# adjo0043/Mathematical-Modeling-Of-Infectious-Diseases-V1

Measured on AMD Instinct MI355X. Metric: ODE-solve+likelihood evals/sec (SEPAIHRD 4-age, 400d), higher is better.
Workload: dtype f64

## Files before the change

### mathematical-modeling-of-infectious-diseases-v1_amd/csrc/phase_pass.py

```python
#!/usr/bin/env python3
import argparse, os, re, subprocess, sys, tempfile

LLVM = "/opt/rocm/lib/llvm/bin"
MCPU = "gfx950"
E64_OK = re.compile(r"^\s+(v_fmac_f64_e32|v_mov_b32_e32|v_mov_b64_e32|v_add_u32_e32|v_sub_u32_e32|v_subrev_u32_e32|v_mul_f32_e32|v_add_f32_e32|"
                    r"v_cvt_f32_f64_e32|v_cvt_f64_f32_e32|v_cvt_f64_i32_e32|v_rcp_f64_e32|v_log_f32_e32|v_exp_f32_e32|v_and_b32_e32|v_or_b32_e32|"
                    r"v_lshlrev_b32_e32|v_max_i32_e32|v_min_i32_e32)\b")


def assemble_sizes(path):
    tmp = tempfile.mkdtemp(prefix="pp_")
    obj = os.path.join(tmp, "a.o")
    subprocess.run([LLVM + "/clang", "-x", "assembler", "-target", "amdgcn-amd-amdhsa", "-mcpu=" + MCPU, "-c", path, "-o", obj], check=True,
                   stdout=subprocess.DEVNULL, stderr=subprocess.DEVNULL)
    dis = subprocess.run([LLVM + "/llvm-objdump", "-d", obj], check=True, capture_output=True, text=True).stdout
    out, cur = {}, None
    for line in dis.splitlines():
        m = re.match(r"^[0-9a-f]+ <(\S+)>:", line)
        if m:
            cur = out.setdefault(m.group(1), [])
            continue
        m = re.match(r"^\s+(\S+).*//\s*([0-9A-Fa-f]+):\s+((?:[0-9A-Fa-f]{8}\s*)+)", line)
        if m and cur is not None:
            cur.append((int(m.group(2), 16), 4 * len(m.group(3).split()), m.group(1)))
    return out


def protected_spans(lines, idxs):
    out = set()
    for k, li in enumerate(idxs):
        if not lines[li].strip().startswith("s_getpc_b64"):
            continue
        last = k
        for m in range(k + 1, min(k + 8, len(idxs))):
            if "@rel32" in lines[idxs[m]]:
                last = m
        out.update(range(k + 1, last + 1))
    return out


def off_phase_runs(sizes, wanted, min_run, min_block):
    n_runs = n_off = 0
    for name, ins in sizes.items():
        if not any(w in name for w in wanted):
            continue
        start = 0
        for k in range(len(ins) + 1):
            if not (k == len(ins) or ins[k][2].startswith(("s_cbranch", "s_branch", "s_endpgm", "s_setpc"))):
                continue
            blk = ins[start:min(k + 1, len(ins))]
            start = k + 1
            if len(blk) < min_block:
                continue
            j = 0
            while j < len(blk):
                if blk[j][1] != 8:
                    j += 1
                    continue
                r = j
                while r < len(blk) and blk[r][1] == 8:
                    r += 1
                if r - j >= min_run:
                    n_runs += 1
                    n_off += blk[j][0] % 8 == 4
                j = r
    return n_runs, n_off


def is_instruction(line):
    t = line.strip()
    return bool(t) and not t.startswith((";", ".", "//", "#")) and not re.match(r"^[\w.$]+:", t)


def main():
    global LLVM, MCPU
    ap = argparse.ArgumentParser()
    ap.add_argument("src"); ap.add_argument("dst")
    ap.add_argument("--kernels", default="sepaihrd_eval_quad_kernel,sepaihrd_eval_kernelILi16E")
    ap.add_argument("--min-run", type=int, default=3)
    ap.add_argument("--min-block", type=int, default=200)
    ap.add_argument("--nop-run", type=int, default=7, help="insert s_nop 0 in front of an off-phase run at least this long when nothing can be re-encoded")
    ap.add_argument("--look-back", type=int, default=12)
    ap.add_argument("--body-residue", type=int, default=-1,
                    help="0, 8, .., 56: pad the ENTRY of every sepaihrd_eval_quad_kernel (s_nop pairs, executed once per wave) so that its "
                         "largest straight-line block -- the common RK body -- starts at this offset within a 64-byte line.  The 8-byte phase "
                         "is untouched (pads come in pairs).  Measured (round 4, tools/ab.sh): five instructions fewer in the consumer's "
                         "logarithm moved the body from offset 60 to 20 and cost the headline kernel 1 % at an unchanged phase report")
    ap.add_argument("--llvm", default=LLVM, help="directory of clang / llvm-objdump")
    ap.add_argument("--mcpu", default=MCPU)
    args = ap.parse_args()
    LLVM, MCPU = args.llvm, args.mcpu
    wanted = args.kernels.split(",")
    sizes = assemble_sizes(args.src)
    lines = open(args.src).read().split("\n")
    func, funcs = None, {}
    for i, l in enumerate(lines):
        m = re.match(r"^(\w+):\s*(;.*)?$", l)
        if m and m.group(1) in sizes:
            func = m.group(1); funcs[func] = []
            continue
        if l.startswith("\t.end_amdhsa_kernel") or l.strip().startswith(".Lfunc_end"):
            func = None
        if func is not None and is_instruction(l):
            funcs[func].append(i)
    n_re = n_nop = n_runs = n_fixed = 0
    edits = {}
    inserts = {}
    for name, idxs in funcs.items():
        if not any(w in name for w in wanted):
            continue
        ins = sizes[name]
        if len(ins) != len(idxs):
            print(f"skip {name[:70]}: {len(ins)} disassembled vs {len(idxs)} listed instructions", file=sys.stderr)
            continue
        guarded = protected_spans(lines, idxs)
        start = 0
        shift = 0
        for k in range(len(ins) + 1):
            end_block = k == len(ins) or ins[k][2].startswith(("s_cbranch", "s_branch", "s_endpgm", "s_setpc"))
            if not end_block:
                continue
            blk = list(range(start, min(k + 1, len(ins))))
            start = k + 1
            if len(blk) < args.min_block:
                continue
            j = 0
            last_touch = -1
            while j < len(blk):
                a = blk[j]
                if ins[a][1] != 8:
                    j += 1
                    continue
                r = j
                while r < len(blk) and ins[blk[r]][1] == 8:
                    r += 1
                run_len = r - j
                if run_len >= args.min_run:
                    n_runs += 1
                    if (ins[a][0] + shift) % 8 == 4:
                        fixed = False
                        for b in range(j - 1, max(j - 1 - args.look_back, last_touch), -1):
                            li = idxs[blk[b]]
                            if blk[b] in guarded:
                                continue
                            if ins[blk[b]][1] == 4 and li not in edits and E64_OK.match(lines[li]) and "0x" not in lines[li] and "dpp" not in lines[li] and "sdwa" not in lines[li]:
                                edits[li] = lines[li].replace("_e32", "_e64", 1)
                                shift += 4; n_re += 1; fixed = True; last_touch = b
                                break
                        if not fixed and run_len >= args.nop_run and a not in guarded:
                            inserts[idxs[a]] = "\ts_nop 0"
                            shift += 4; n_nop += 1; fixed = True; last_touch = j
                        n_fixed += fixed
                j = r
    out = []
    for i, l in enumerate(lines):
        if i in inserts:
            out.append(inserts[i])
        out.append(edits.get(i, l))
    open(args.dst, "w").write("\n".join(out))
    try:
        after = assemble_sizes(args.dst)
    except subprocess.CalledProcessError:
        print("phase_pass: the rewritten assembly does not assemble", file=sys.stderr)
        sys.exit(1)
    if args.body_residue >= 0:
        out_lines = open(args.dst).read().split("\n")
        inserts_at = {}
        for name, ins in after.items():
            if "sepaihrd_eval_quad_kernel" not in name or not ins:
                continue
            blocks, start = [], 0
            for k in range(len(ins) + 1):
                if k == len(ins) or ins[k][2].startswith(("s_cbranch", "s_branch", "s_endpgm", "s_setpc")):
                    blocks.append(ins[start:min(k + 1, len(ins))]); start = k + 1
            bodies = [b for b in blocks if len(b) >= args.min_block and sum(1 for _, _, m in b if "f64" in m or "dpp" in m) * 2 > len(b)]
            if not bodies:
                continue
            body = min(bodies, key=len)
            delta = (args.body_residue - body[0][0]) % 64
            delta -= delta % 8
            if delta:
                inserts_at[name] = delta // 4
        if inserts_at:
            padded = []
            for l in out_lines:
                padded.append(l)
                m = re.match(r"^(\w+):\s*(;.*)?$", l)
                if m and m.group(1) in inserts_at:
                    padded.extend(["\ts_nop 0"] * inserts_at[m.group(1)])
            open(args.dst, "w").write("\n".join(padded))
            try:
                after = assemble_sizes(args.dst)
            except subprocess.CalledProcessError:
                print("phase_pass: the padded assembly does not assemble", file=sys.stderr)
                sys.exit(1)
            print(f"body residue {args.body_residue}: entry pads {sorted(set(inserts_at.values()))} s_nop in {len(inserts_at)} kernels")
    runs_before, off_before = off_phase_runs(sizes, wanted, args.min_run, args.min_block)
    runs_after, off_after = off_phase_runs(after, wanted, args.min_run, args.min_block)
    print(f"runs of >= {args.min_run} wide encodings: {n_runs}; off phase and fixed: {n_fixed} ({n_re} re-encoded, {n_nop} s_nop); "
          f"off-phase runs by the assembled addresses: {off_before} of {runs_before} before, {off_after} of {runs_after} after")
    if off_after > off_before:
        print("phase_pass: the rewritten assembly has MORE off-phase runs than its input", file=sys.stderr)
        sys.exit(1)


if __name__ == "__main__":
    main()
```

### mathematical-modeling-of-infectious-diseases-v1_amd/csrc/sepaihrd_kernels.hip

```cpp
#include <hip/hip_runtime.h>
#include <float.h>
#include <math.h>
#include <stdint.h>
#include <stdlib.h>

#include <mutex>
#include <utility>

#include "sepaihrd_device.h"

#ifndef SEPAIHRD_DOPRI5_WPS2
#define SEPAIHRD_DOPRI5_WPS2 0
#endif
#ifndef SEPAIHRD_LL_STATE_IN_LDS
#define SEPAIHRD_LL_STATE_IN_LDS 1
#endif
#ifndef SEPAIHRD_ARITH_FMA
#error "compile with -DSEPAIHRD_ARITH_FMA=0 or 1"
#endif

namespace sepaihrd {
namespace {

#include "sepaihrd_dev_common.inc"
// ... 91 lines not shown
    dx[3] = fma(-q.get(MF_GAMMA_A), A, q.get(MF_PG) * P);
    dx[4] = fma(-q.get(MF_R_I), I, q.get(MF_PI) * P);
    dx[5] = fma(-q.get(MF_R_H), H, flow_IH);
    dx[6] = fma(-q.get(MF_R_ICU), ICU, flow_H_ICU);
    dx[7] = fma(q.get(MF_GAMMA_ICU), ICU, fma(q.get(MF_GAMMA_A), A, fma(q.get(MF_GAMMA_H), H, q.get(MF_GAMMA_I) * I)));
    dx[8] = fma(q.get(MF_D_ICU), ICU, fma(q.get(MF_D_COMM), I, q.get(MF_D_H) * H));
    dx[9] = flow_IH;
    dx[10] = flow_H_ICU;
#else
    const double flow_EP = q.get(MF_SIGMA) * E;
    const double flow_P_out = q.get(MF_GAMMA_P) * P;
    const double flow_PA = q.get(MF_P) * flow_P_out;
    const double flow_PI = flow_P_out - flow_PA;
    const double flow_IH = q.get(MF_H) * I;
    const double flow_IR = q.get(MF_GAMMA_I) * I;
    const double flow_ID_community = q.get(MF_D_COMM) * I;
    const double flow_H_ICU = q.get(MF_ICU) * H;

    dx[0] = -flow_SE;
    dx[1] = flow_SE - flow_EP;
    dx[2] = flow_EP - flow_P_out;
    dx[3] = flow_PA - q.get(MF_GAMMA_A) * A;
    const double I_out = flow_IR + flow_IH + flow_ID_community;
    const double H_out = q.get(MF_GAMMA_H) * H + q.get(MF_D_H) * H + flow_H_ICU;
    const double ICU_out = (q.get(MF_GAMMA_ICU) + q.get(MF_D_ICU)) * ICU;
    dx[4] = flow_PI - I_out;
    dx[5] = flow_IH - H_out;
    dx[6] = flow_H_ICU - ICU_out;
    dx[7] = q.get(MF_GAMMA_A) * A + flow_IR + q.get(MF_GAMMA_H) * H + q.get(MF_GAMMA_ICU) * ICU;
    dx[8] = q.get(MF_D_H) * H + q.get(MF_D_ICU) * ICU + flow_ID_community;
    dx[9] = flow_IH;
    dx[10] = flow_H_ICU;
#endif
}

#ifdef SEPAIHRD_STAMPS
#define SEP_STAMP(var)                                                                 \
    do {                                                                               \
        __builtin_amdgcn_sched_barrier(0);                                             \
        asm volatile("s_memtime %0\n\ts_waitcnt lgkmcnt(0)" : "=s"(var)::"memory");     \
        __builtin_amdgcn_sched_barrier(0);                                             \
    } while (0)
#else
#define SEP_STAMP(var) do { } while (0)
#endif

#include "sepaihrd_step_control.inc"

#if SEPAIHRD_ARITH_FMA
enum QuadCoefDopri5 { QD_B32 = 0, QD_B42, QD_B43, QD_B52, QD_B53, QD_B54, QD_B62, QD_B63, QD_B64, QD_B65, QD_C3, QD_C4, QD_C5,
                      QD_C6, QD_DC4, QD_DC5, QD_DC6 , QD_DC7  };
enum QuadCoefCashKarp { QK_A32 = 0, QK_A42, QK_A43, QK_A52, QK_A53, QK_A54, QK_A62, QK_A63, QK_A64, QK_A65, QK_B3, QK_B4, QK_B6,
                        QK_DB4, QK_DB5, QK_DB6 };
__device__ const double QUAD_COEF[2][2][16] = {
    {{dp::b32, dp::b42, dp::b43, dp::b52, dp::b53, dp::b54, dp::b62, dp::b63, dp::b64, dp::b65, dp::c3, dp::c4, dp::c5, dp::c6,
      dp::dc4, dp::dc5},
     {dp::dc6, dp::dc7, 0, 0, 0, 0, 0, 0, 0, 0, 0, 0, 0, 0, 0, 0}},
    {{ck::a32, ck::a42, ck::a43, ck::a52, ck::a53, ck::a54, ck::a62, ck::a63, ck::a64, ck::a65, ck::b3, ck::b4, ck::b6, ck::db4,
      ck::db5, ck::db6},
     {0, 0, 0, 0, 0, 0, 0, 0, 0, 0, 0, 0, 0, 0, 0, 0}}};
template <int IDX>
__device__ __forceinline__ void stage_term(double& acc, double vecA, double vecB, double k) {
    if constexpr (IDX < 16) fmac_row_bcast<IDX, 0xf, false>(acc, vecA, k);
    else fmac_row_bcast<IDX - 16, 0xf, false>(acc, vecB, k);
}


#ifndef SEPAIHRD_FMA16_STAGE_PADS
#define SEPAIHRD_FMA16_STAGE_PADS 194
#endif
#ifndef SEPAIHRD_FMA3_STAGE_PADS
#define SEPAIHRD_FMA3_STAGE_PADS 0
#endif
#define SEP_ROW_STAGE_PAD(i, v) do { if ((((N == NUM_COMP) ? SEPAIHRD_FMA16_STAGE_PADS : (N == 3) ? SEPAIHRD_FMA3_STAGE_PADS : 0) >> (i)) & 1) asm volatile("s_nop 0" : "+v"(v)); } while (0)

template <int SOLVER, int N, class RHS>
__device__ __forceinline__ void rk_stages_row_coef(const double cur, const double vecA, const double vecB, const double (&x)[N],
                                                   double (&k1)[N], double (&k2)[N], double (&k3)[N], double (&k4)[N], double (&k5)[N],
                                                   double (&k6)[N], double (&k7)[N], double (&xnew)[N], double (&xerr)[N],
                                                   const double (&bks)[7], RHS&& rhs_call) {
    double xt[N];
        if (SOLVER == 0) {
            { const double f1 = cur * dp::b21;
              SEP_UNROLL for (int c = 0; c < N; ++c) xt[c] = fma(f1, k1[c], x[c]);
              SEP_ROW_STAGE_PAD(0, xt[0]); rhs_call(xt, k2, bks[1]); }
            SEP_ROW_STAGE_PAD(1, k2[0]);
            { const double f1 = cur * dp::b31;
              SEP_UNROLL for (int c = 0; c < N; ++c) { xt[c] = fma(f1, k1[c], x[c]); stage_term<QD_B32>(xt[c], vecA, vecB, k2[c]); }
              SEP_ROW_STAGE_PAD(2, xt[0]); rhs_call(xt, k3, bks[2]); }
            SEP_ROW_STAGE_PAD(3, k3[0]);
            { const double f1 = cur * dp::b41;
              SEP_UNROLL for (int c = 0; c < N; ++c) {
                  xt[c] = fma(f1, k1[c], x[c]); stage_term<QD_B42>(xt[c], vecA, vecB, k2[c]); stage_term<QD_B43>(xt[c], vecA, vecB, k3[c]); }
              SEP_ROW_STAGE_PAD(4, xt[0]); rhs_call(xt, k4, bks[3]); }
            SEP_ROW_STAGE_PAD(5, k4[0]);
            { const double f1 = cur * dp::b51;
              SEP_UNROLL for (int c = 0; c < N; ++c) {
                  xt[c] = fma(f1, k1[c], x[c]); stage_term<QD_B52>(xt[c], vecA, vecB, k2[c]); stage_term<QD_B53>(xt[c], vecA, vecB, k3[c]);
                  stage_term<QD_B54>(xt[c], vecA, vecB, k4[c]); }
              SEP_ROW_STAGE_PAD(6, xt[0]); rhs_call(xt, k5, bks[4]); }
            SEP_ROW_STAGE_PAD(7, k5[0]);
            { const double f1 = cur * dp::b61;
              SEP_UNROLL for (int c = 0; c < N; ++c) {
                  xt[c] = fma(f1, k1[c], x[c]); stage_term<QD_B62>(xt[c], vecA, vecB, k2[c]); stage_term<QD_B63>(xt[c], vecA, vecB, k3[c]);
                  stage_term<QD_B64>(xt[c], vecA, vecB, k4[c]); stage_term<QD_B65>(xt[c], vecA, vecB, k5[c]); }
              SEP_ROW_STAGE_PAD(8, xt[0]); rhs_call(xt, k6, bks[5]); }
            SEP_ROW_STAGE_PAD(9, k6[0]);
            { const double f1 = cur * dp::c1;
              SEP_UNROLL for (int c = 0; c < N; ++c) {
                  xnew[c] = fma(f1, k1[c], x[c]); stage_term<QD_C3>(xnew[c], vecA, vecB, k3[c]); stage_term<QD_C4>(xnew[c], vecA, vecB, k4[c]);
                  stage_term<QD_C5>(xnew[c], vecA, vecB, k5[c]); stage_term<QD_C6>(xnew[c], vecA, vecB, k6[c]); }
              SEP_ROW_STAGE_PAD(10, xnew[0]); rhs_call(xnew, k7, bks[6]); }
            SEP_ROW_STAGE_PAD(11, k7[0]);
            { const double e1 = cur * dp::dc1, e3 = cur * dp::dc3;
              SEP_UNROLL for (int c = 0; c < N; ++c) {
                  xerr[c] = fma(e1, k1[c], e3 * k3[c]); stage_term<QD_DC4>(xerr[c], vecA, vecB, k4[c]); stage_term<QD_DC5>(xerr[c], vecA, vecB, k5[c]);
                  stage_term<QD_DC6>(xerr[c], vecA, vecB, k6[c]); stage_term<QD_DC7>(xerr[c], vecA, vecB, k7[c]); } }
        } else {
            rhs_call(x, k1, bks[0]);
            { const double f1 = ck::a21 * cur;
              SEP_UNROLL for (int c = 0; c < N; ++c) xt[c] = fma(f1, k1[c], x[c]);
              rhs_call(xt, k2, bks[1]); }
            { const double f1 = ck::a31 * cur;
              SEP_UNROLL for (int c = 0; c < N; ++c) { xt[c] = fma(f1, k1[c], x[c]); stage_term<QK_A32>(xt[c], vecA, vecB, k2[c]); }
              rhs_call(xt, k3, bks[2]); }
            { const double f1 = ck::a41 * cur;
              SEP_UNROLL for (int c = 0; c < N; ++c) {
// ... 1040 lines not shown
```

### mathematical-modeling-of-infectious-diseases-v1_amd/csrc/sepaihrd_lane_split.inc

```

constexpr int QUAD_LANES = 16;
constexpr int QUAD_CPW = WAVE / QUAD_LANES;
constexpr int QUAD_SLOTS = 3;

template <int CTRL>
__device__ __forceinline__ double quad_rot(double v) { return dpp_move<CTRL>(v); }
constexpr int QROT_LEFT = 0x93;
constexpr int QROT_NEXT = 0x39;

#ifndef SEPAIHRD_STRICT_STAGE_PADS
#define SEPAIHRD_STRICT_STAGE_PADS 0
#endif
#define SEP_STAGE_PAD(i, v) do { if ((SEPAIHRD_STRICT_STAGE_PADS >> (i)) & 1) asm volatile("s_nop 0" : "+v"(v)); } while (0)
#ifndef SEPAIHRD_STRICT_HEAD_PADS_CK
#define SEPAIHRD_STRICT_HEAD_PADS_CK 0
#endif
#ifndef SEPAIHRD_STRICT_STAGE_PADS_CK
#define SEPAIHRD_STRICT_STAGE_PADS_CK 0
#endif
#define SEP_STAGE_PAD_CK(i, v) do { if ((SEPAIHRD_STRICT_STAGE_PADS_CK >> (i)) & 1) asm volatile("s_nop 0" : "+v"(v)); } while (0)
#define SEP_PHASE_PAD(n) do { if ((n) >= 1) asm volatile("s_nop 0"); if ((n) >= 2) asm volatile("s_nop 0"); if ((n) >= 3) asm volatile("s_nop 0"); } while (0)
using lanemask = unsigned long long;
__device__ __forceinline__ lanemask lanes_where(bool p) { return __builtin_amdgcn_ballot_w64(p); }
__device__ __forceinline__ bool lane_of(lanemask m) { return __builtin_amdgcn_inverse_ballot_w64(m); }
__device__ __forceinline__ double min_plain(double a, double b) {
    double r;
    asm("v_min_f64 %0, %1, %2" : "=v"(r) : "v"(a), "v"(b));
    return r;
}

#if SEPAIHRD_ARITH_FMA
struct QuadModel {
    double theta_inf, m[4];
    double cO1, cL1;
    double cO0, cX0, cL0;
    double a1, a2, a3, a4, a5;
};

__device__ __forceinline__ void rhs_quad(const QuadModel& q, const double (&x)[QUAD_SLOTS], double (&dx)[QUAD_SLOTS],
                                         double beta_eff) {
    const double Lx1 = quad_rot<QROT_LEFT>(x[1]);
    const double Nx1 = quad_rot<QROT_NEXT>(x[1]), Nx0 = quad_rot<QROT_NEXT>(x[0]);
    const double pressure = fma(q.theta_inf, x[1], Lx1 + x[0]);
    double lambda = 0.0;
    fmac_row_bcast<2, 0xf, true>(lambda, pressure, q.m[0]);
    fmac_row_bcast<6, 0xf, false>(lambda, pressure, q.m[1]);
    fmac_row_bcast<10, 0xf, false>(lambda, pressure, q.m[2]);
    fmac_row_bcast<14, 0xf, false>(lambda, pressure, q.m[3]);
    lambda *= beta_eff;
    const double lambda_val = (0.0 < lambda) ? lambda : 0.0;
    const double W = lambda_val * x[0];
    dx[1] = fma(q.cO1, x[1], fma(q.cL1, Lx1, W));
    dx[0] = fma(q.cO0, x[0], fma(q.cX0, x[1], fma(q.cL0, Lx1, -W)));
    dx[2] = fma(q.a5, Nx0, fma(q.a4, x[0], fma(q.a3, Lx1, fma(q.a2, Nx1, q.a1 * x[1]))));
}

#else
struct QuadModel {
    double theta_inf, h_infec, inv_N, a_i, m[4];
    double u2, u3, v1, v2, v3;
    double u5, u6, u7, w1;
    double q1, q2, q3, q4, q5, q6;
};

__device__ __forceinline__ void rhs_quad(const QuadModel& q, const double (&x)[QUAD_SLOTS], double (&dx)[QUAD_SLOTS],
                                         double beta_eff) {
    const double Lx1 = quad_rot<QROT_LEFT>(x[1]);
    const double Nx1 = quad_rot<QROT_NEXT>(x[1]), Nx0 = quad_rot<QROT_NEXT>(x[0]);
    const double total_inf = Lx1 + x[0] + q.theta_inf * x[1];
    const double pressure = total_inf * q.h_infec * q.inv_N;
    double lambda = q.m[0] * dpp_bcast_row<2, 0xf, 2, 0x0>(pressure);
    lambda += q.m[1] * dpp_bcast_row<6, 0xf, 6, 0x0>(pressure);
    lambda += q.m[2] * dpp_bcast_row<10, 0xf, 10, 0x0>(pressure);
    lambda += q.m[3] * dpp_bcast_row<14, 0xf, 14, 0x0>(pressure);
    lambda *= beta_eff * q.a_i;
    const double lambda_val = (0.0 < lambda) ? lambda : 0.0;
    const double W = lambda_val * x[0];
    {
        const double t = q.u2 * Lx1;
        const double flow_in = (W + t) - q.u3 * t;
        const double out = q.v1 * x[1] + q.v2 * x[1] + q.v3 * x[1];
        dx[1] = flow_in - out;
    }
    {
        const double t5 = q.u5 * Lx1;
        const double flow_in = q.u6 * t5 + q.u7 * x[1];
        dx[0] = (flow_in - q.w1 * x[0]) - W;
    }
    dx[2] = q.q1 * x[0] + q.q2 * x[1] + q.q3 * Nx1 + q.q4 * Nx0 + q.q5 * x[0] + q.q6 * Lx1;
}

#endif

__device__ __forceinline__ int quad_comp(int cg, int slot) {
    if (slot == 0) return cg == 0 ? 0 : (cg == 1 ? -1 : (cg == 2 ? 3 : 6));
    if (slot == 1) return cg == 0 ? 1 : (cg == 1 ? 2 : (cg == 2 ? 4 : 5));
    return cg == 0 ? 10 : (cg == 1 ? 9 : (cg == 2 ? 7 : 8));
}

constexpr int QUAD_RING = 32;
constexpr int QUAD_BURST = 12;
constexpr int QUAD_UNITS = 4;
constexpr int QUAD_ROW_DOUBLES = QUAD_CPW * 12;
constexpr int QUAD_SPIN_LIMIT = 1 << 22;
constexpr size_t QUAD_FUSED_MAX_LDS = 144 * 1024;
constexpr int QUAD_CTRL_INTS = 8 + QUAD_UNITS * (2 * QUAD_CPW + 1 + 3 * QUAD_CPW);
constexpr int SEPAIHRD_STATUS_PIPELINE = 4;
// ... 364 lines not shown
            } else {
                if (stores) *cum_row = v - prev;
                cum_row += cum_step;
            }
            prev = v;
            if constexpr (TRAJ) {
            if (out.traj != nullptr && chain_valid && age < n_real) {
                double* tdst = out.traj + ((size_t)chain * pb.T + k) * (NUM_COMP * n_real) + age;
                SEP_UNROLL
                for (int s = 0; s < NS; ++s) {
                    const int c = quad_comp(cg, s);
                    if (c >= 0) tdst[c * n_real] = x[s];
                }
            }
            }
        }
    };

    int k_next = 1;
    double t = pb.times[0];
    double dt = pb.dt_hint;
    int fails = 0;
    int attempts = 0;
    double t_next = (T > 1) ? pb.times[1] : t;
    double t_after = (T > 2) ? pb.times[2] : t_next;
    observe_store(act, 0);
    if (T <= 1) act = 0ull;

    sch.lo = INFINITY; sch.hi = -INFINITY; sch.bk = 0.0;
    double k1[NS];
    if (SOLVER == 0) {
        int c0, c1;
        segment_index2(sch, pb.nm_pad, t, t, c0, c1);
        rhs_quad(q, x, k1, sch.bkv[c0]);
    }
    const double eps_abs = pb.abs_tol, eps_rel = pb.rel_tol;
#if SEPAIHRD_ARITH_FMA
    const double coefA = QUAD_COEF[SOLVER][0][lane & 15], coefB = QUAD_COEF[SOLVER][1][lane & 15];
#else
    const double coefA = STRICT_QUAD_COEF[SOLVER][0][lane & 15], coefB = STRICT_QUAD_COEF[SOLVER][1][lane & 15];
#endif

#ifdef SEPAIHRD_STAMPS
    unsigned long long st0 = 0, st1 = 0, st2 = 0, st3 = 0, st4 = 0;
    unsigned long long acc_head = 0, acc_body = 0, acc_err = 0, acc_tail = 0;
#endif
    auto attempt = [&](const double cur, const double vecA, const double vecB, const double (&bks)[7]) __attribute__((always_inline)) {
        const bool active = lane_of(act);
        (void)active;
        SEP_STAMP(st1);
        double k2[NS], k3[NS], k4[NS], k5[NS], k6[NS], k7[NS];
        double xnew[NS], xerr[NS];
#if SEPAIHRD_ARITH_FMA
        rk_stages_row_coef<SOLVER, NS>(cur, vecA, vecB, x, k1, k2, k3, k4, k5, k6, k7, xnew, xerr, bks,
                                       [&](const double (&xin)[NS], double (&kout)[NS], double bk) { rhs_quad(q, xin, kout, bk); });
#else
        double xt[NS];
        if (SOLVER == 0) {
            { const double f1 = strict_coef<SD_B21>(vecA, vecB);
              SEP_UNROLL for (int c = 0; c < NS; ++c) xt[c] = x[c] + f1 * k1[c];
              rhs_quad(q, xt, k2, bks[1]); }
            SEP_STAGE_PAD(0, k2[0]);
            { const double f1 = strict_coef<SD_B31>(vecA, vecB), f2 = strict_coef<SD_B32>(vecA, vecB);
              SEP_UNROLL for (int c = 0; c < NS; ++c) xt[c] = x[c] + f1 * k1[c] + f2 * k2[c];
              rhs_quad(q, xt, k3, bks[2]); }
            SEP_STAGE_PAD(1, k3[0]);
            { const double f1 = strict_coef<SD_B41>(vecA, vecB), f2 = strict_coef<SD_B42>(vecA, vecB), f3 = strict_coef<SD_B43>(vecA, vecB);
              SEP_UNROLL for (int c = 0; c < NS; ++c) xt[c] = x[c] + f1 * k1[c] + f2 * k2[c] + f3 * k3[c];
              rhs_quad(q, xt, k4, bks[3]); }
            SEP_STAGE_PAD(2, k4[0]);
            { const double f1 = strict_coef<SD_B51>(vecA, vecB), f2 = strict_coef<SD_B52>(vecA, vecB), f3 = strict_coef<SD_B53>(vecA, vecB), f4 = strict_coef<SD_B54>(vecA, vecB);
              SEP_UNROLL for (int c = 0; c < NS; ++c)
                  xt[c] = x[c] + f1 * k1[c] + f2 * k2[c] + f3 * k3[c] + f4 * k4[c];
              rhs_quad(q, xt, k5, bks[4]); }
            SEP_STAGE_PAD(3, k5[0]);
            { const double f1 = strict_coef<SD_B61>(vecA, vecB), f2 = strict_coef<SD_B62>(vecA, vecB), f3 = strict_coef<SD_B63>(vecA, vecB), f4 = strict_coef<SD_B64>(vecA, vecB),
                           f5 = strict_coef<SD_B65>(vecA, vecB);
              SEP_UNROLL for (int c = 0; c < NS; ++c)
                  xt[c] = x[c] + f1 * k1[c] + f2 * k2[c] + f3 * k3[c] + f4 * k4[c] + f5 * k5[c];
              rhs_quad(q, xt, k6, bks[5]); }
            SEP_STAGE_PAD(4, k6[0]);
            { const double f1 = strict_coef<SD_C1>(vecA, vecB), f3 = strict_coef<SD_C3>(vecA, vecB), f4 = strict_coef<SD_C4>(vecA, vecB), f5 = strict_coef<SD_C5>(vecA, vecB),
                           f6 = strict_coef<SD_C6>(vecA, vecB);
              SEP_UNROLL for (int c = 0; c < NS; ++c)
                  xnew[c] = x[c] + f1 * k1[c] + f3 * k3[c] + f4 * k4[c] + f5 * k5[c] + f6 * k6[c];
              rhs_quad(q, xnew, k7, bks[6]); }
            SEP_STAGE_PAD(5, k7[0]);
            { const double e1 = strict_coef<SD_DC1>(vecA, vecB), e3 = strict_coef<SD_DC3>(vecA, vecB), e4 = strict_coef<SD_DC4>(vecA, vecB), e5 = strict_coef<SD_DC5>(vecA, vecB),
                           e6 = strict_coef<SD_DC6>(vecA, vecB), e7 = strict_coef<SD_DC7>(vecA, vecB);
              SEP_UNROLL for (int c = 0; c < NS; ++c)
                  xerr[c] = e1 * k1[c] + e3 * k3[c] + e4 * k4[c] + e5 * k5[c] + e6 * k6[c] + e7 * k7[c]; }
        } else {
            rhs_quad(q, x, k1, bks[0]);
            SEP_STAGE_PAD_CK(0, k1[0]);
            { const double f1 = strict_coef<SK_A21>(vecA, vecB);
              SEP_UNROLL for (int c = 0; c < NS; ++c) xt[c] = x[c] + f1 * k1[c];
              rhs_quad(q, xt, k2, bks[1]); }
            SEP_STAGE_PAD_CK(1, k2[0]);
            { const double f1 = strict_coef<SK_A31>(vecA, vecB), f2 = strict_coef<SK_A32>(vecA, vecB);
              SEP_UNROLL for (int c = 0; c < NS; ++c) xt[c] = x[c] + f1 * k1[c] + f2 * k2[c];
              rhs_quad(q, xt, k3, bks[2]); }
            SEP_STAGE_PAD_CK(2, k3[0]);
            { const double f1 = strict_coef<SK_A41>(vecA, vecB), f2 = strict_coef<SK_A42>(vecA, vecB), f3 = strict_coef<SK_A43>(vecA, vecB);
              SEP_UNROLL for (int c = 0; c < NS; ++c) xt[c] = x[c] + f1 * k1[c] + f2 * k2[c] + f3 * k3[c];
              rhs_quad(q, xt, k4, bks[3]); }
            SEP_STAGE_PAD_CK(3, k4[0]);
            { const double f1 = strict_coef<SK_A51>(vecA, vecB), f2 = strict_coef<SK_A52>(vecA, vecB), f3 = strict_coef<SK_A53>(vecA, vecB), f4 = strict_coef<SK_A54>(vecA, vecB);
              SEP_UNROLL for (int c = 0; c < NS; ++c)
// ... 51 lines not shown
            const double cur_after = lane_of(dec_m | inc_m) ? cur * f : cur;
            dt = rej ? cur_after : (acc ? max_moved(dt, cur_after) : dt);
            n_rej += rej ? 1 : 0;
            const lanemask gave_up = dec_m & lanes_where(fails >= 500);
            if (lane_of(gave_up)) status = 2;
            act &= ~gave_up;
            fails = acc ? 0 : fails + (rej ? 1 : 0);
        } else {
            fails = 0;
        }
        n_acc += acc ? 1 : 0;
        SEP_STAMP(st3);
        {
            if (acc) {
                t += cur;
                SEP_UNROLL
                for (int c = 0; c < NS; ++c) x[c] = xnew[c];
                if (SOLVER == 0) {
                    SEP_UNROLL
                    for (int c = 0; c < NS; ++c) k1[c] = k7[c];
                }
            }
            const lanemask reached_m = acc_m & ~lanes_where((t_next - t) > DBL_EPSILON);
            if (__builtin_expect(reached_m != 0ull, 1)) {
                const double t_fetch = lds_times[(k_next + 2 < T) ? k_next + 2 : T - 1];
                observe_store(reached_m, k_next);
                if (lane_of(reached_m)) {
                    t = t_next;
                    ++k_next;
                    t_next = t_after;
                    t_after = t_fetch;
                }
                act &= ~(reached_m & lanes_where(k_next >= T));
            }
        }
        SEP_STAMP(st4);
    };
    while (act != 0ull && attempts < pb.max_attempts) {
#ifdef SEPAIHRD_PHASE_NOPS_HEAD
        SEP_PHASE_PAD(SEPAIHRD_PHASE_NOPS_HEAD);
#endif
#if !SEPAIHRD_ARITH_FMA
        if constexpr (SOLVER == 1) SEP_PHASE_PAD(SEPAIHRD_STRICT_HEAD_PADS_CK);
#endif
        SEP_STAMP(st0);
        double cur_m;
        {
            const double gap = t_next - t;
            asm volatile("v_min_f64 %0, %1, %2" : "=v"(cur_m) : "v"(dt), "v"(gap));
        }
        const double cur = lane_of(act) ? cur_m : 1.0;
#if SEPAIHRD_ARITH_FMA
        double vecA, vecB;
        asm("v_mul_f64 %0, %2, %3\n\tv_mul_f64 %1, %2, %4" : "=&v"(vecA), "=&v"(vecB) : "v"(cur), "v"(coefA), "v"(coefB));
#else
        const double vecA = cur * coefA, vecB = cur * coefB;
#endif
        const double tmin = (SOLVER == 0) ? fma(cur, dp::a2, t) : t;
        const double tmax = (SOLVER == 0) ? t + cur : fma(ck::c5, cur, t);
        const lanemask in_seg = lanes_where(tmin > sch.lo) & lanes_where(tmax <= sch.hi);
        auto stage_values = [&](double (&bks)[7], int c_lo, int c_hi, double v_lo, double v_hi) __attribute__((always_inline)) {
            double tau[7];
            if (SOLVER == 0) {
                tau[0] = t;
                tau[1] = t + cur * dp::a2; tau[2] = t + cur * dp::a3; tau[3] = t + cur * dp::a4;
                tau[4] = t + cur * dp::a5; tau[5] = t + cur; tau[6] = t + cur;
            } else {
                tau[0] = t;
                tau[1] = t + ck::c2 * cur; tau[2] = t + ck::c3 * cur; tau[3] = t + ck::c4 * cur;
                tau[4] = t + ck::c5 * cur; tau[5] = t + ck::c6 * cur; tau[6] = t + cur;
            }
            if (lanes_where(c_hi > c_lo + 1) == 0ull) {
                const double bpt = (c_lo < pb.nm) ? sch.me[c_lo] : INFINITY;
                SEP_UNROLL
                for (int s = 0; s < 7; ++s) bks[s] = (tau[s] > bpt) ? v_hi : v_lo;
            } else {
                for (int s = 0; s < 7; ++s) {
                    int ca, cb;
                    segment_index2(sch, pb.nm_pad, tau[s], tau[s], ca, cb);
                    bks[s] = sch.bkv[ca];
                }
            }
        };
#if SEPAIHRD_ARITH_FMA
        if (__builtin_expect((act & ~in_seg) != 0ull, 0)) {
            int c_lo, c_hi;
            segment_index2(sch, pb.nm_pad, tmin, tmax, c_lo, c_hi);
            const double v_lo = sch.bkv[c_lo], v_hi = sch.bkv[c_hi];
            const lanemask straddles = act & lanes_where(c_hi > c_lo);
            sch.lo = (c_hi > 0) ? sch.me[c_hi - 1] : -INFINITY;
            sch.hi = (c_hi < pb.nm) ? sch.me[c_hi] : INFINITY;
            sch.bk = v_hi;
            if (straddles != 0ull) {
                double bks[7];
                stage_values(bks, c_lo, c_hi, v_lo, v_hi);
                __builtin_amdgcn_s_waitcnt(0xc07f);
                attempt(cur, vecA, vecB, bks);
                continue;
            }
            __builtin_amdgcn_s_waitcnt(0xc07f);
        }
        const double one_value[7] = {sch.bk, sch.bk, sch.bk, sch.bk, sch.bk, sch.bk, sch.bk};
        attempt(cur, vecA, vecB, one_value);
#else
        double bks[7];
        if (__builtin_expect((act & ~in_seg) != 0ull, 0)) {
            int c_lo, c_hi;
// ... 96 lines not shown
```

Before: 8.480 million.

## Hand-schedule quad RK stages with DPP broadcast coefficients and exact phase padding

Adds a dedicated quad RK stage routine that folds the leading stage coefficients into the DPP-broadcast coefficient table. Each stage now uses inline-asm fmac_dpp chains, and the contact sum is fused with the neighbour rotation and the next stage's first term. The phase pass gains a dynamic-programming choice of e64 widenings and s_nop inserts per block, meant to keep runs of 8-byte instructions 8-byte aligned. The intent is fewer issued instructions and fewer instruction-fetch alignment stalls in the FP64 RK body, at the cost of fragile hand-written asm and a risk of numerical reordering.

```diff
diff --git a/mathematical-modeling-of-infectious-diseases-v1_amd/csrc/phase_pass.py b/mathematical-modeling-of-infectious-diseases-v1_amd/csrc/phase_pass.py
--- a/mathematical-modeling-of-infectious-diseases-v1_amd/csrc/phase_pass.py
+++ b/mathematical-modeling-of-infectious-diseases-v1_amd/csrc/phase_pass.py
@@ -72,6 +72,53 @@
     return bool(t) and not t.startswith((";", ".", "//", "#")) and not re.match(r"^[\w.$]+:", t)
 
 
+def best_choices(blk, ins, shift, can_widen, can_pad, min_run, nop_run):
+    n = len(blk)
+    wide = [ins[a][1] == 8 for a in blk]
+    run_len = [0] * n
+    in_run = [False] * n
+    j = 0
+    while j < n:
+        if not wide[j]:
+            j += 1
+            continue
+        r = j
+        while r < n and wide[r]:
+            r += 1
+        run_len[j] = r - j
+        if r - j >= min_run:
+            for x in range(j, r):
+                in_run[x] = True
+        j = r
+    INF = float("inf")
+    cost = [[INF, INF] for _ in range(n + 1)]
+    pick = [[None, None] for _ in range(n + 1)]
+    cost[n] = [0, 0]
+    for i in range(n - 1, -1, -1):
+        off0 = (ins[blk[i]][0] + shift) % 8 == 4
+        for t in (0, 1):
+            options = []
+            for pad in ((0, 1) if wide[i] and run_len[i] >= nop_run and can_pad[i] else (0,)):
+                tt = t ^ pad
+                off = off0 ^ bool(tt)
+                if wide[i]:
+                    options.append((43 * pad + (0 if not off else 11 if in_run[i] else 5) + cost[i + 1][tt], (pad, 0)))
+                else:
+                    options.append((cost[i + 1][tt], (0, 0)))
+                    if can_widen[i]:
+                        options.append(((11 if off else 0) + 0.01 + cost[i + 1][tt ^ 1], (0, 1)))
+            cost[i][t], pick[i][t] = min(options)
+    widen, pads, t = [], [], 0
+    for i in range(n):
+        pad, w = pick[i][t]
+        if pad:
+            pads.append(i)
+        if w:
+            widen.append(i)
+        t ^= pad ^ w
+    return widen, pads
+
+
 def main():
     global LLVM, MCPU
     ap = argparse.ArgumentParser()
@@ -79,8 +126,17 @@
     ap.add_argument("--kernels", default="sepaihrd_eval_quad_kernel,sepaihrd_eval_kernelILi16E")
     ap.add_argument("--min-run", type=int, default=3)
     ap.add_argument("--min-block", type=int, default=200)
-    ap.add_argument("--nop-run", type=int, default=7, help="insert s_nop 0 in front of an off-phase run at least this long when nothing can be re-encoded")
+    ap.add_argument("--nop-run", type=int, default=0,
+                    help="insert s_nop 0 in front of an off-phase run at least this long when nothing can be re-encoded (0: 7 for the walk, 4 for the exact choice)")
     ap.add_argument("--look-back", type=int, default=12)
+    ap.add_argument("--greedy", action="store_true",
+                    help="the round-3 walk (nearest re-encodable instruction within --look-back in front of each off-phase run) for EVERY "
+                         "kernel: what the strict build was placed and measured with")
+    ap.add_argument("--exact-kernels", default="sepaihrd_eval_quad_kernel",
+                    help="without --greedy: the kernels (substrings) whose blocks get the exact choice (best_choices); the other --kernels "
+                         "keep the walk -- the 16-age kernel's code is what it was before the exact choice existed")
+    ap.add_argument("--common-body", choices=["walk", "exact"], default="walk",
+                    help="how the common RK body of an --exact-kernels kernel (the shortest of its big FP64 blocks) is treated")
     ap.add_argument("--body-residue", type=int, default=-1,
                     help="0, 8, .., 56: pad the ENTRY of every sepaihrd_eval_quad_kernel (s_nop pairs, executed once per wave) so that its "
                          "largest straight-line block -- the common RK body -- starts at this offset within a 64-byte line.  The 8-byte phase "
@@ -90,6 +146,7 @@
     ap.add_argument("--mcpu", default=MCPU)
     args = ap.parse_args()
     LLVM, MCPU = args.llvm, args.mcpu
+    exact_names = [] if args.greedy else [w for w in args.exact_kernels.split(",") if w]
     wanted = args.kernels.split(",")
     sizes = assemble_sizes(args.src)
     lines = open(args.src).read().split("\n")
@@ -114,6 +171,18 @@
             print(f"skip {name[:70]}: {len(ins)} disassembled vs {len(idxs)} listed instructions", file=sys.stderr)
             continue
         guarded = protected_spans(lines, idxs)
+        exact = any(w in name for w in exact_names)
+        nop_run = args.nop_run if args.nop_run > 0 else 7
+        common_start = -1
+        if exact:
+            bodies, b0 = [], 0
+            for k in range(len(ins) + 1):
+                if k == len(ins) or ins[k][2].startswith(("s_cbranch", "s_branch", "s_endpgm", "s_setpc")):
+                    b = range(b0, min(k + 1, len(ins))); b0 = k + 1
+                    if len(b) >= args.min_block and sum(1 for x in b if "f64" in ins[x][2] or "dpp" in ins[x][2]) * 2 > len(b):
+                        bodies.append(b)
+            if bodies:
+                common_start = min(bodies, key=len)[0]
         start = 0
         shift = 0
         for k in range(len(ins) + 1):
@@ -123,6 +192,18 @@
             blk = list(range(start, min(k + 1, len(ins))))
             start = k + 1
             if len(blk) < args.min_block:
+                continue
+            is_common = exact and blk[0] == common_start
+            if exact and not (is_common and args.common_body == "walk"):
+                pad_run = args.nop_run if args.nop_run > 0 else (7 if is_common else 4)
+                can_widen = [ins[x][1] == 4 and x not in guarded and bool(E64_OK.match(lines[idxs[x]])) and "0x" not in lines[idxs[x]]
+                             and "dpp" not in lines[idxs[x]] and "sdwa" not in lines[idxs[x]] for x in blk]
+                widen, pads = best_choices(blk, ins, shift, can_widen, [x not in guarded for x in blk], args.min_run, pad_run)
+                for i in widen:
+                    edits[idxs[blk[i]]] = lines[idxs[blk[i]]].replace("_e32", "_e64", 1)
+                for i in pads:
+                    inserts[idxs[blk[i]]] = "\ts_nop 0"
+                shift += 4 * (len(widen) + len(pads)); n_re += len(widen); n_nop += len(pads)
                 continue
             j = 0
             last_touch = -1
@@ -147,7 +228,7 @@
                                 edits[li] = lines[li].replace("_e32", "_e64", 1)
                                 shift += 4; n_re += 1; fixed = True; last_touch = b
                                 break
-                        if not fixed and run_len >= args.nop_run and a not in guarded:
+                        if not fixed and run_len >= nop_run and a not in guarded:
                             inserts[idxs[a]] = "\ts_nop 0"
                             shift += 4; n_nop += 1; fixed = True; last_touch = j
                         n_fixed += fixed
@@ -177,8 +258,10 @@
             if not bodies:
                 continue
             body = min(bodies, key=len)
-            delta = (args.body_residue - body[0][0]) % 64
-            delta -= delta % 8
+            delta = (args.body_residue + (body[0][0] - args.body_residue) % 8 - body[0][0]) % 64
+            if args.greedy:
+                delta = (args.body_residue - body[0][0]) % 64
+                delta -= delta % 8
             if delta:
                 inserts_at[name] = delta // 4
         if inserts_at:
@@ -197,8 +280,9 @@
             print(f"body residue {args.body_residue}: entry pads {sorted(set(inserts_at.values()))} s_nop in {len(inserts_at)} kernels")
     runs_before, off_before = off_phase_runs(sizes, wanted, args.min_run, args.min_block)
     runs_after, off_after = off_phase_runs(after, wanted, args.min_run, args.min_block)
-    print(f"runs of >= {args.min_run} wide encodings: {n_runs}; off phase and fixed: {n_fixed} ({n_re} re-encoded, {n_nop} s_nop); "
-          f"off-phase runs by the assembled addresses: {off_before} of {runs_before} before, {off_after} of {runs_after} after")
+    head = (f"runs of >= {args.min_run} wide encodings: {n_runs}; off phase and fixed: {n_fixed} ({n_re} re-encoded, {n_nop} s_nop); " if not exact_names else
+            f"walk: {n_fixed} of {n_runs} runs fixed; exact choice per block (with the walk's): {n_re} re-encoded, {n_nop} s_nop; ")
+    print(head + f"off-phase runs by the assembled addresses: {off_before} of {runs_before} before, {off_after} of {runs_after} after")
     if off_after > off_before:
         print("phase_pass: the rewritten assembly has MORE off-phase runs than its input", file=sys.stderr)
         sys.exit(1)
diff --git a/mathematical-modeling-of-infectious-diseases-v1_amd/csrc/sepaihrd_kernels.hip b/mathematical-modeling-of-infectious-diseases-v1_amd/csrc/sepaihrd_kernels.hip
--- a/mathematical-modeling-of-infectious-diseases-v1_amd/csrc/sepaihrd_kernels.hip
+++ b/mathematical-modeling-of-infectious-diseases-v1_amd/csrc/sepaihrd_kernels.hip
@@ -167,13 +167,14 @@
                       QD_C6, QD_DC4, QD_DC5, QD_DC6 , QD_DC7  };
 enum QuadCoefCashKarp { QK_A32 = 0, QK_A42, QK_A43, QK_A52, QK_A53, QK_A54, QK_A62, QK_A63, QK_A64, QK_A65, QK_B3, QK_B4, QK_B6,
                         QK_DB4, QK_DB5, QK_DB6 };
+enum QuadLeadCoef { QL_STAGE2 = 2, QL_STAGE3, QL_STAGE4, QL_STAGE5, QL_STAGE6, QL_NEW, QL_ERR1, QL_ERR3 };
 __device__ const double QUAD_COEF[2][2][16] = {
     {{dp::b32, dp::b42, dp::b43, dp::b52, dp::b53, dp::b54, dp::b62, dp::b63, dp::b64, dp::b65, dp::c3, dp::c4, dp::c5, dp::c6,
       dp::dc4, dp::dc5},
-     {dp::dc6, dp::dc7, 0, 0, 0, 0, 0, 0, 0, 0, 0, 0, 0, 0, 0, 0}},
+     {dp::dc6, dp::dc7, dp::b21, dp::b31, dp::b41, dp::b51, dp::b61, dp::c1, dp::dc1, dp::dc3, 0, 0, 0, 0, 0, 0}},
     {{ck::a32, ck::a42, ck::a43, ck::a52, ck::a53, ck::a54, ck::a62, ck::a63, ck::a64, ck::a65, ck::b3, ck::b4, ck::b6, ck::db4,
       ck::db5, ck::db6},
-     {0, 0, 0, 0, 0, 0, 0, 0, 0, 0, 0, 0, 0, 0, 0, 0}}};
+     {0, 0, ck::a21, ck::a31, ck::a41, ck::a51, ck::a61, ck::b1, ck::db1, ck::db3, 0, 0, 0, 0, 0, 0}}};
 template <int IDX>
 __device__ __forceinline__ void stage_term(double& acc, double vecA, double vecB, double k) {
     if constexpr (IDX < 16) fmac_row_bcast<IDX, 0xf, false>(acc, vecA, k);
@@ -184,10 +185,7 @@
 #ifndef SEPAIHRD_FMA16_STAGE_PADS
 #define SEPAIHRD_FMA16_STAGE_PADS 194
 #endif
-#ifndef SEPAIHRD_FMA3_STAGE_PADS
-#define SEPAIHRD_FMA3_STAGE_PADS 0
-#endif
-#define SEP_ROW_STAGE_PAD(i, v) do { if ((((N == NUM_COMP) ? SEPAIHRD_FMA16_STAGE_PADS : (N == 3) ? SEPAIHRD_FMA3_STAGE_PADS : 0) >> (i)) & 1) asm volatile("s_nop 0" : "+v"(v)); } while (0)
+#define SEP_ROW_STAGE_PAD(i, v) do { if ((((N == NUM_COMP) ? SEPAIHRD_FMA16_STAGE_PADS : 0) >> (i)) & 1) asm volatile("s_nop 0" : "+v"(v)); } while (0)
 
 template <int SOLVER, int N, class RHS>
 __device__ __forceinline__ void rk_stages_row_coef(const double cur, const double vecA, const double vecB, const double (&x)[N],
diff --git a/mathematical-modeling-of-infectious-diseases-v1_amd/csrc/sepaihrd_lane_split.inc b/mathematical-modeling-of-infectious-diseases-v1_amd/csrc/sepaihrd_lane_split.inc
--- a/mathematical-modeling-of-infectious-diseases-v1_amd/csrc/sepaihrd_lane_split.inc
+++ b/mathematical-modeling-of-infectious-diseases-v1_amd/csrc/sepaihrd_lane_split.inc
@@ -37,22 +37,142 @@
     double a1, a2, a3, a4, a5;
 };
 
-__device__ __forceinline__ void rhs_quad(const QuadModel& q, const double (&x)[QUAD_SLOTS], double (&dx)[QUAD_SLOTS],
-                                         double beta_eff) {
+template <bool WANT2>
+__device__ __forceinline__ void contact_sum(const QuadModel& q, const double x1, const double lx1_plus_x0, double& lambda, double& Nx1,
+                                            double& fill, const double fa, const double fb, const double fc) {
+    double pressure = lx1_plus_x0;
+    if constexpr (WANT2) {
+        int lo, hi;
+        asm("v_fmac_f64_e32 %0, %4, %5\n\t"
+            "v_mov_b64_e32 %1, 0\n\t"
+            "v_mov_b32_dpp %2, %6 quad_perm:[1,2,3,0] row_mask:0xf bank_mask:0xf bound_ctrl:1\n\t"
+            "v_fmac_f64_dpp %1, %0, %8 row_newbcast:2 row_mask:0xf bank_mask:0xf\n\t"
+            "v_mov_b32_dpp %3, %7 quad_perm:[1,2,3,0] row_mask:0xf bank_mask:0xf bound_ctrl:1\n\t"
+            "v_fmac_f64_dpp %1, %0, %9 row_newbcast:6 row_mask:0xf bank_mask:0xf\n\t"
+            "v_fmac_f64_dpp %1, %0, %10 row_newbcast:10 row_mask:0xf bank_mask:0xf\n\t"
+            "v_fmac_f64_dpp %1, %0, %11 row_newbcast:14 row_mask:0xf bank_mask:0xf"
+            : "+v"(pressure), "=&v"(lambda), "=&v"(lo), "=&v"(hi)
+            : "v"(q.theta_inf), "v"(x1), "v"(__double2loint(x1)), "v"(__double2hiint(x1)), "v"(q.m[0]), "v"(q.m[1]), "v"(q.m[2]), "v"(q.m[3]));
+        Nx1 = __hiloint2double(hi, lo);
+    } else {
+        asm("v_fmac_f64_e32 %0, %3, %4\n\t"
+            "v_mov_b64_e32 %1, 0\n\t"
+            "v_fma_f64 %2, %9, %10, %11\n\t"
+            "v_fmac_f64_dpp %1, %0, %5 row_newbcast:2 row_mask:0xf bank_mask:0xf\n\t"
+            "v_fmac_f64_dpp %1, %0, %6 row_newbcast:6 row_mask:0xf bank_mask:0xf\n\t"
+            "v_fmac_f64_dpp %1, %0, %7 row_newbcast:10 row_mask:0xf bank_mask:0xf\n\t"
+            "v_fmac_f64_dpp %1, %0, %8 row_newbcast:14 row_mask:0xf bank_mask:0xf"
+            : "+v"(pressure), "=&v"(lambda), "=&v"(fill)
+            : "v"(q.theta_inf), "v"(x1), "v"(q.m[0]), "v"(q.m[1]), "v"(q.m[2]), "v"(q.m[3]), "v"(fa), "v"(fb), "v"(fc));
+        Nx1 = 0.0;
+    }
+}
+
+template <bool WANT2>
+__device__ __forceinline__ void rhs_quad_body(const QuadModel& q, const double (&x)[QUAD_SLOTS], double (&dx)[QUAD_SLOTS],
+                                              double beta_eff, double& fill, const double fa, const double fb, const double fc) {
     const double Lx1 = quad_rot<QROT_LEFT>(x[1]);
-    const double Nx1 = quad_rot<QROT_NEXT>(x[1]), Nx0 = quad_rot<QROT_NEXT>(x[0]);
-    const double pressure = fma(q.theta_inf, x[1], Lx1 + x[0]);
-    double lambda = 0.0;
-    fmac_row_bcast<2, 0xf, true>(lambda, pressure, q.m[0]);
-    fmac_row_bcast<6, 0xf, false>(lambda, pressure, q.m[1]);
-    fmac_row_bcast<10, 0xf, false>(lambda, pressure, q.m[2]);
-    fmac_row_bcast<14, 0xf, false>(lambda, pressure, q.m[3]);
+    const double Nx0 = quad_rot<QROT_NEXT>(x[0]);
+    double lambda, Nx1;
+    contact_sum<WANT2>(q, x[1], Lx1 + x[0], lambda, Nx1, fill, fa, fb, fc);
     lambda *= beta_eff;
     const double lambda_val = (0.0 < lambda) ? lambda : 0.0;
     const double W = lambda_val * x[0];
     dx[1] = fma(q.cO1, x[1], fma(q.cL1, Lx1, W));
     dx[0] = fma(q.cO0, x[0], fma(q.cX0, x[1], fma(q.cL0, Lx1, -W)));
-    dx[2] = fma(q.a5, Nx0, fma(q.a4, x[0], fma(q.a3, Lx1, fma(q.a2, Nx1, q.a1 * x[1]))));
+    if constexpr (WANT2) dx[2] = fma(q.a5, Nx0, fma(q.a4, x[0], fma(q.a3, Lx1, fma(q.a2, Nx1, q.a1 * x[1]))));
+    else dx[2] = 0.0;
+}
+__device__ __forceinline__ void rhs_quad(const QuadModel& q, const double (&x)[QUAD_SLOTS], double (&dx)[QUAD_SLOTS], double beta_eff) {
+    double unused = 0.0;
+    rhs_quad_body<true>(q, x, dx, beta_eff, unused, 0.0, 0.0, 0.0);
+}
+__device__ __forceinline__ double rhs_quad_slots01_fill(const QuadModel& q, const double (&x)[QUAD_SLOTS], double (&dx)[QUAD_SLOTS],
+                                                        double beta_eff, const double fa, const double fb, const double fc) {
+    double fill;
+    rhs_quad_body<false>(q, x, dx, beta_eff, fill, fa, fb, fc);
+    return fill;
+}
+
+#define SEP_QLINE(t, s) "v_fmac_f64_dpp %[a" #s "], %[v" #t "], %[w" #t #s "] row_newbcast:%[n" #t "] row_mask:0xf bank_mask:0xf\n\t"
+#define SEP_QTERM2(t) SEP_QLINE(t, 1) SEP_QLINE(t, 0)
+#define SEP_QTERM3(t) SEP_QLINE(t, 1) SEP_QLINE(t, 0) SEP_QLINE(t, 2)
+#define SEP_QIN2(t, IDX, k) [v##t] "v"((IDX) < 16 ? vecA : vecB), [n##t] "n"((IDX) & 15), [w##t##1] "v"(k[1]), [w##t##0] "v"(k[0])
+#define SEP_QIN3(t, IDX, k) SEP_QIN2(t, IDX, k), [w##t##2] "v"(k[2])
+#define SEP_QACC2(acc) [a1] "+v"(acc[1]), [a0] "+v"(acc[0])
+#define SEP_QACC3(acc) SEP_QACC2(acc), [a2] "+v"(acc[2])
+
+template <int IDX>
+__device__ __forceinline__ double lead(double vecB) { return dpp_bcast_row<IDX, 0xf, IDX, 0x0>(vecB); }
+
+template <int SOLVER>
+__device__ __forceinline__ void rk_stages_quad(const QuadModel& q, const double vecA, const double vecB, const double (&x)[QUAD_SLOTS],
+                                               double (&k1)[QUAD_SLOTS], double (&k2)[QUAD_SLOTS], double (&k3)[QUAD_SLOTS],
+                                               double (&k4)[QUAD_SLOTS], double (&k5)[QUAD_SLOTS], double (&k6)[QUAD_SLOTS],
+                                               double (&k7)[QUAD_SLOTS], double (&xnew)[QUAD_SLOTS], double (&xerr)[QUAD_SLOTS],
+                                               const double (&bks)[7]) {
+    double xt[QUAD_SLOTS];
+    xt[2] = 0.0;
+    auto first_term = [&](double (&acc)[QUAD_SLOTS], double f1, int slots) {
+        acc[0] = fma(f1, k1[0], x[0]);
+        acc[1] = fma(f1, k1[1], x[1]);
+        if (slots == 3) acc[2] = fma(f1, k1[2], x[2]);
+    };
+    if (SOLVER == 0) {
+        first_term(xt, lead<QL_STAGE2>(vecB), 2);
+        {
+            const double f1 = lead<QL_STAGE3>(vecB);
+            const double xt1 = rhs_quad_slots01_fill(q, xt, k2, bks[1], f1, k1[1], x[1]);
+            xt[0] = fma(f1, k1[0], x[0]);
+            xt[1] = xt1;
+        }
+        asm(SEP_QTERM2(1) : SEP_QACC2(xt) : SEP_QIN2(1, QD_B32, k2));
+        rhs_quad(q, xt, k3, bks[2]);
+        first_term(xt, lead<QL_STAGE4>(vecB), 2);
+        asm(SEP_QTERM2(1) SEP_QTERM2(2) : SEP_QACC2(xt) : SEP_QIN2(1, QD_B42, k2), SEP_QIN2(2, QD_B43, k3));
+        rhs_quad(q, xt, k4, bks[3]);
+        first_term(xt, lead<QL_STAGE5>(vecB), 2);
+        asm(SEP_QTERM2(1) SEP_QTERM2(2) SEP_QTERM2(3) : SEP_QACC2(xt) : SEP_QIN2(1, QD_B52, k2), SEP_QIN2(2, QD_B53, k3), SEP_QIN2(3, QD_B54, k4));
+        rhs_quad(q, xt, k5, bks[4]);
+        first_term(xt, lead<QL_STAGE6>(vecB), 2);
+        asm(SEP_QTERM2(1) SEP_QTERM2(2) SEP_QTERM2(3) SEP_QTERM2(4)
+            : SEP_QACC2(xt) : SEP_QIN2(1, QD_B62, k2), SEP_QIN2(2, QD_B63, k3), SEP_QIN2(3, QD_B64, k4), SEP_QIN2(4, QD_B65, k5));
+        rhs_quad(q, xt, k6, bks[5]);
+        first_term(xnew, lead<QL_NEW>(vecB), 3);
+        asm(SEP_QTERM3(1) SEP_QTERM3(2) SEP_QTERM3(3) SEP_QTERM3(4)
+            : SEP_QACC3(xnew) : SEP_QIN3(1, QD_C3, k3), SEP_QIN3(2, QD_C4, k4), SEP_QIN3(3, QD_C5, k5), SEP_QIN3(4, QD_C6, k6));
+        rhs_quad(q, xnew, k7, bks[6]);
+        const double e1 = lead<QL_ERR1>(vecB), e3 = lead<QL_ERR3>(vecB);
+        SEP_UNROLL for (int c = 0; c < QUAD_SLOTS; ++c) xerr[c] = fma(e1, k1[c], e3 * k3[c]);
+        asm(SEP_QTERM3(1) SEP_QTERM3(2) SEP_QTERM3(3) SEP_QTERM3(4)
+            : SEP_QACC3(xerr) : SEP_QIN3(1, QD_DC4, k4), SEP_QIN3(2, QD_DC5, k5), SEP_QIN3(3, QD_DC6, k6), SEP_QIN3(4, QD_DC7, k7));
+    } else {
+        rhs_quad(q, x, k1, bks[0]);
+        first_term(xt, lead<QL_STAGE2>(vecB), 2);
+        {
+            const double f1 = lead<QL_STAGE3>(vecB);
+            const double xt1 = rhs_quad_slots01_fill(q, xt, k2, bks[1], f1, k1[1], x[1]);
+            xt[0] = fma(f1, k1[0], x[0]);
+            xt[1] = xt1;
+        }
+        asm(SEP_QTERM2(1) : SEP_QACC2(xt) : SEP_QIN2(1, QK_A32, k2));
+        rhs_quad(q, xt, k3, bks[2]);
+        first_term(xt, lead<QL_STAGE4>(vecB), 2);
+        asm(SEP_QTERM2(1) SEP_QTERM2(2) : SEP_QACC2(xt) : SEP_QIN2(1, QK_A42, k2), SEP_QIN2(2, QK_A43, k3));
+        rhs_quad(q, xt, k4, bks[3]);
+        first_term(xt, lead<QL_STAGE5>(vecB), 2);
+        asm(SEP_QTERM2(1) SEP_QTERM2(2) SEP_QTERM2(3) : SEP_QACC2(xt) : SEP_QIN2(1, QK_A52, k2), SEP_QIN2(2, QK_A53, k3), SEP_QIN2(3, QK_A54, k4));
+        rhs_quad(q, xt, k5, bks[4]);
+        first_term(xt, lead<QL_STAGE6>(vecB), 2);
+        asm(SEP_QTERM2(1) SEP_QTERM2(2) SEP_QTERM2(3) SEP_QTERM2(4)
+            : SEP_QACC2(xt) : SEP_QIN2(1, QK_A62, k2), SEP_QIN2(2, QK_A63, k3), SEP_QIN2(3, QK_A64, k4), SEP_QIN2(4, QK_A65, k5));
+        rhs_quad(q, xt, k6, bks[5]);
+        first_term(xnew, lead<QL_NEW>(vecB), 3);
+        asm(SEP_QTERM3(1) SEP_QTERM3(2) SEP_QTERM3(3) : SEP_QACC3(xnew) : SEP_QIN3(1, QK_B3, k3), SEP_QIN3(2, QK_B4, k4), SEP_QIN3(3, QK_B6, k6));
+        const double e1 = lead<QL_ERR1>(vecB), e3 = lead<QL_ERR3>(vecB);
+        SEP_UNROLL for (int c = 0; c < QUAD_SLOTS; ++c) xerr[c] = fma(e3, k3[c], e1 * k1[c]);
+        asm(SEP_QTERM3(1) SEP_QTERM3(2) SEP_QTERM3(3) : SEP_QACC3(xerr) : SEP_QIN3(1, QK_DB4, k4), SEP_QIN3(2, QK_DB5, k5), SEP_QIN3(3, QK_DB6, k6));
+    }
 }
 
 #else
@@ -523,8 +643,7 @@
         double k2[NS], k3[NS], k4[NS], k5[NS], k6[NS], k7[NS];
         double xnew[NS], xerr[NS];
 #if SEPAIHRD_ARITH_FMA
-        rk_stages_row_coef<SOLVER, NS>(cur, vecA, vecB, x, k1, k2, k3, k4, k5, k6, k7, xnew, xerr, bks,
-                                       [&](const double (&xin)[NS], double (&kout)[NS], double bk) { rhs_quad(q, xin, kout, bk); });
+        rk_stages_quad<SOLVER>(q, vecA, vecB, x, k1, k2, k3, k4, k5, k6, k7, xnew, xerr, bks);
 #else
         double xt[NS];
         if (SOLVER == 0) {
@@ -682,7 +801,7 @@
         const double cur = lane_of(act) ? cur_m : 1.0;
 #if SEPAIHRD_ARITH_FMA
         double vecA, vecB;
-        asm("v_mul_f64 %0, %2, %3\n\tv_mul_f64 %1, %2, %4" : "=&v"(vecA), "=&v"(vecB) : "v"(cur), "v"(coefA), "v"(coefB));
+        asm("v_mul_f64 %1, %2, %4\n\tv_mul_f64 %0, %2, %3" : "=&v"(vecA), "=&v"(vecB) : "v"(cur), "v"(coefA), "v"(coefB));
 #else
         const double vecA = cur * coefA, vecB = cur * coefB;
 #endif
```

After: 8.695 million, median of 6. +2.5%, better.
